# yidingjiang/action_conditioned_GANs

Hardware: AMD Instinct MI355X
Metric: GAN train steps/sec (G+D) on 64x64x3xT=8 push seq (higher is better)
Workload: dtype f32; 1 GPU; BASELINE config 2 per GPU: batch=32 64x64x3 T=8 --adv --loss bce --dna (k=5) --opt adam fp32; global_batch=32, n_critic=1, parallelism=dp1, hip_graphs=True, bn_grid_exchange=on, lookahead=True, opt=adam, trace_run=False, step_executions=1380

## Files before the change

action_conditioned_gans_amd/csrc/dna.hip:

```cpp
#include <hip/hip_runtime.h>

#include <type_traits>

#include "common.h"

namespace {

constexpr int TX = 64;

struct Second {
  void* ptr;
  int pitch, off, half;
};
__device__ __forceinline__ void second_store(const Second& s2, long long pix, int c, float v) {
  if (s2.half) reinterpret_cast<__bf16*>(s2.ptr)[pix * s2.pitch + s2.off + c] = (__bf16)v;
  else reinterpret_cast<float*>(s2.ptr)[pix * s2.pitch + s2.off + c] = v;
}
__device__ __forceinline__ void second_store_pixel(const Second& s2, long long pix, int C, const float* img_c, const float (&f)[4]) {
  if (C == 3 && s2.off == 3 && s2.pitch == 8) {
    if (s2.half) {
      typedef __bf16 bf8v __attribute__((ext_vector_type(8)));
      const bf8v v = {(__bf16)img_c[0], (__bf16)img_c[1], (__bf16)img_c[2], (__bf16)f[0], (__bf16)f[1], (__bf16)f[2], (__bf16)0.f, (__bf16)0.f};
      *reinterpret_cast<bf8v*>(reinterpret_cast<__bf16*>(s2.ptr) + pix * 8) = v;
    } else {
      float4* o = reinterpret_cast<float4*>(reinterpret_cast<float*>(s2.ptr) + pix * 8);
      o[0] = make_float4(img_c[0], img_c[1], img_c[2], f[0]);
      o[1] = make_float4(f[1], f[2], 0.f, 0.f);
    }
    return;
  }
  for (int c = 0; c < C; ++c) second_store(s2, pix, c, f[c]);
}
__device__ __forceinline__ float second_load(const Second& s2, long long pix, int c) {
  return s2.half ? (float)reinterpret_cast<const __bf16*>(s2.ptr)[pix * s2.pitch + s2.off + c]
                 : reinterpret_cast<const float*>(s2.ptr)[pix * s2.pitch + s2.off + c];
}

template <typename TL>
__host__ __device__ constexpr int logit_pitch(int kk) { return sizeof(TL) == 2 ? (kk + 7) & ~7 : kk; }

template <int K, int TY, bool BWD, int CC, typename TL>
__global__ __launch_bounds__(TX* TY) void dna_kernel(const TL* __restrict__ logits, const float* __restrict__ bias,
                                                     const float* __restrict__ img, const float* __restrict__ dout,
                                                     void* __restrict__ outv, float* __restrict__ bpart, int H, int W, int Crt,
                                                     const Second s2) {
  constexpr int KK = K * K, S = KK | 1, NT = TX * TY, P = (K - 1) / 2, LP = logit_pitch<TL>(KK);
  constexpr int WW = TX + K - 1, WH = TY + K - 1;
  constexpr bool F32 = sizeof(TL) == 4;
  __shared__ __attribute__((aligned(16))) float lg[NT * S];
  __shared__ float win[WH * WW * 4];
  __shared__ float bs[KK];
  const int C = CC ? CC : Crt;
  float* const out = reinterpret_cast<float*>(outv);
  TL* const dlog = reinterpret_cast<TL*>(outv);

  const int tid = threadIdx.x;
  const int x0 = blockIdx.x * TX, y0 = blockIdx.y * TY, b = blockIdx.z;
  const int txv = min(TX, W - x0);
  if (tid < KK) bs[tid] = bias ? bias[tid] : 0.f;

  for (int wy = tid / 64; wy < WH; wy += NT / 64) {
    const int y = y0 - P + wy;
    const bool yok = y >= 0 && y < H;
    const long long rowbase = (long long)(b * H + (yok ? y : 0)) * W * C;
    for (int f = tid % 64; f < WW * C; f += 64) {
      const int gx = (x0 - P) * C + f;
      win[wy * WW * C + f] = (yok && gx >= 0 && gx < W * C) ? img[rowbase + gx] : 0.f;
    }
  }
  const long long pix0 = (long long)(b * H + y0) * W + x0;
  const bool vec = F32 && (S == KK) && ((pix0 * KK) % 4 == 0) && (((long long)W * KK) % 4 == 0) && ((txv * KK) % 4 == 0) &&
                   ((reinterpret_cast<uintptr_t>(logits) & 15) == 0);
  if constexpr (F32) {
    if (vec) {
      const int span4 = txv * KK / 4;
      for (int ty = 0; ty < TY; ++ty) {
        if (y0 + ty >= H) break;
        const float4* src = reinterpret_cast<const float4*>(logits + (pix0 + (long long)ty * W) * KK);
        float4* dst = reinterpret_cast<float4*>(lg + ty * TX * S);
        for (int i = tid; i < span4; i += NT) dst[i] = src[i];
      }
    } else {
      for (int idx = tid; idx < TY * TX * KK; idx += NT) {
        const int ty = idx / (TX * KK), e = idx - ty * (TX * KK);
        if (y0 + ty < H && e < txv * KK) lg[(ty * TX + e / KK) * S + e % KK] = acg::ldf(logits + (pix0 + (long long)ty * W) * KK + e);
      }
    }
  } else {
    constexpr int Q = LP / 4;
    for (int idx = tid; idx < TY * TX * Q; idx += NT) {
      const int ty = idx / (TX * Q), e = idx - ty * (TX * Q), px = e / Q, q = e - px * Q;
      if (y0 + ty < H && px < txv && 4 * q < KK) {
        float v[4];
        acg::ldv<4>(logits + (pix0 + (long long)ty * W + px) * LP + 4 * q, v);
        float* d = lg + (ty * TX + px) * S + 4 * q;
#pragma unroll
        for (int u = 0; u < 4; ++u)
          if (4 * q + u < KK) d[u] = v[u];
      }
    }
  }
  __syncthreads();

  const int ty = tid / TX, tx = tid - ty * TX;
  const int y = y0 + ty, x = x0 + tx;
  const bool valid = y < H && x < W;
  float* l = lg + tid * S;
  const float* wbase = win + (ty * WW + tx) * C;

  if (valid) {
    float v[KK];
#pragma unroll
    for (int t = 0; t < KK; ++t) v[t] = l[t] + bs[t];
    float mx = v[0];
#pragma unroll
    for (int t = 1; t < KK; ++t) mx = fmaxf(mx, v[t]);
    const long long pix = (long long)(b * H + y) * W + x;
    if constexpr (!BWD) {
      float den = 0.f, a0 = 0.f, a1 = 0.f, a2 = 0.f, a3 = 0.f;
#pragma unroll
      for (int i = 0; i < K; ++i)
#pragma unroll
        for (int j = 0; j < K; ++j) {
          const float e = __expf(v[i * K + j] - mx);
          const float* wp = wbase + (i * WW + j) * C;
          den += e;
          a0 += e * wp[0];
          if (C > 1) a1 += e * wp[1];
          if (C > 2) a2 += e * wp[2];
          if (C > 3) a3 += e * wp[3];
        }
      const float inv = 1.f / den;
      float* o = out + pix * C;
      o[0] = a0 * inv;
      if (C > 1) o[1] = a1 * inv;
      if (C > 2) o[2] = a2 * inv;
      if (C > 3) o[3] = a3 * inv;
      if (s2.ptr) {
        const float fr[4] = {a0 * inv, a1 * inv, a2 * inv, a3 * inv};
        second_store_pixel(s2, pix, C, wbase + (P * WW + P) * C, fr);
      }
    } else {
      const float* dO = dout + pix * C;
      float d0 = dO[0], d1 = C > 1 ? dO[1] : 0.f, d2 = C > 2 ? dO[2] : 0.f, d3 = C > 3 ? dO[3] : 0.f;
      if (s2.ptr) {
        d0 += second_load(s2, pix, 0);
        if (C > 1) d1 += second_load(s2, pix, 1);
        if (C > 2) d2 += second_load(s2, pix, 2);
        if (C > 3) d3 += second_load(s2, pix, 3);
      }
      float gv[KK];
      float den = 0.f, dotn = 0.f;
#pragma unroll
      for (int i = 0; i < K; ++i)
#pragma unroll
        for (int j = 0; j < K; ++j) {
          const float* wp = wbase + (i * WW + j) * C;
          float g = d0 * wp[0];
          if (C > 1) g += d1 * wp[1];
          if (C > 2) g += d2 * wp[2];
          if (C > 3) g += d3 * wp[3];
          const float e = __expf(v[i * K + j] - mx);
          gv[i * K + j] = g;
          v[i * K + j] = e;
          den += e;
          dotn += e * g;
        }
      const float inv = 1.f / den, dot = dotn * inv;
#pragma unroll
      for (int t = 0; t < KK; ++t) l[t] = (v[t] * inv) * (gv[t] - dot);
    }
  } else if constexpr (BWD) {
#pragma unroll
    for (int t = 0; t < KK; ++t) l[t] = 0.f;
  }
  if constexpr (BWD) {
    __syncthreads();
    if constexpr (F32) {
      if (vec) {
        const int span4 = txv * KK / 4;
        for (int ty2 = 0; ty2 < TY; ++ty2) {
          if (y0 + ty2 >= H) break;
          float4* dstg = reinterpret_cast<float4*>(dlog + (pix0 + (long long)ty2 * W) * KK);
          const float4* srcl = reinterpret_cast<const float4*>(lg + ty2 * TX * S);
          for (int i = tid; i < span4; i += NT) dstg[i] = srcl[i];
        }
      } else {
        for (int idx = tid; idx < TY * TX * KK; idx += NT) {
          const int ty2 = idx / (TX * KK), e = idx - ty2 * (TX * KK);
          if (y0 + ty2 < H && e < txv * KK) acg::stf(dlog + (pix0 + (long long)ty2 * W) * KK + e, lg[(ty2 * TX + e / KK) * S + e % KK]);
        }
      }
    } else {
      constexpr int Q = LP / 4;
      for (int idx = tid; idx < TY * TX * Q; idx += NT) {
        const int ty2 = idx / (TX * Q), e = idx - ty2 * (TX * Q), px = e / Q, q = e - px * Q;
        if (y0 + ty2 < H && px < txv && 4 * q < KK) {
          const float* sl = lg + (ty2 * TX + px) * S + 4 * q;
          float v[4];
#pragma unroll
          for (int u = 0; u < 4; ++u) v[u] = 4 * q + u < KK ? sl[u] : 0.f;
          acg::stv<4>(dlog + (pix0 + (long long)ty2 * W + px) * LP + 4 * q, v);
        }
      }
    }
    if (bpart) {
      const int t = tid & 31, seg = tid >> 5;
      float sacc = 0.f;
      if (t < KK)
        for (int px = seg * 32; px < seg * 32 + 32; ++px) sacc += lg[px * S + t];
      __syncthreads();
      if (t < KK) win[seg * 32 + t] = sacc;
      __syncthreads();
      if (tid < KK) {
        float tot = 0.f;
        for (int g2 = 0; g2 < NT / 32; ++g2) tot += win[g2 * 32 + tid];
        bpart[(long long)((blockIdx.z * gridDim.y + blockIdx.y) * gridDim.x + blockIdx.x) * KK + tid] = tot;
      }
    }
  }
}

template <int K, bool BWD, int CC, typename TL>
__global__ __launch_bounds__(256) void dna_rows_kernel(const TL* __restrict__ logits, const float* __restrict__ bias,
                                                       const float* __restrict__ img, const float* __restrict__ dout,
                                                       void* __restrict__ outv, float* __restrict__ bpart, int H, int W, int Crt,
                                                       const Second s2) {
  constexpr int E = sizeof(TL) == 2 ? 2 : 1;
  constexpr int KK = K * K, P = (K - 1) / 2, R = (KK + 16 * E - 1) / (16 * E), WW = 64 + K - 1, LP = logit_pitch<TL>(KK);
  const int C = CC ? CC : Crt;
  __shared__ float win[K * WW * 4];
  __shared__ float bsum[BWD ? 16 * R * 16 * E : 1];
  float* const out = reinterpret_cast<float*>(outv);
  TL* const dlog = reinterpret_cast<TL*>(outv);
  const int tid = threadIdx.x, l16 = tid & 15, grp = tid >> 4;
  const int x0 = blockIdx.x * 64, y = blockIdx.y, b = blockIdx.z;
  for (int i = tid; i < K * WW * C; i += 256) {
    const int c = i % C, p = i / C, wx = p % WW, wy = p / WW;
    const int gy = y - P + wy, gx = x0 - P + wx;
    win[i] = (gy >= 0 && gy < H && gx >= 0 && gx < W) ? img[(((long long)b * H + gy) * W + gx) * C + c] : 0.f;
  }
  __syncthreads();
  auto dpp = [](float v, auto ctrl) {
    return __builtin_bit_cast(float, __builtin_amdgcn_update_dpp(0, __builtin_bit_cast(int, v), decltype(ctrl)::value, 0xF, 0xF, false));
  };
  using QP1 = std::integral_constant<int, 0xB1>;
  using QP2 = std::integral_constant<int, 0x4E>;
  using RHM = std::integral_constant<int, 0x141>;
  using RM = std::integral_constant<int, 0x140>;
  auto row_max = [&](float v) {
    v = fmaxf(v, dpp(v, QP1{})); v = fmaxf(v, dpp(v, QP2{})); v = fmaxf(v, dpp(v, RHM{})); v = fmaxf(v, dpp(v, RM{}));
    return v;
  };
  auto row_sum = [&](float v) {
    v += dpp(v, QP1{}); v += dpp(v, QP2{}); v += dpp(v, RHM{}); v += dpp(v, RM{});
    return v;
  };
  int woff[R][E];
  float bia[R][E], bacc[R][E];
#pragma unroll
  for (int r = 0; r < R; ++r)
#pragma unroll
    for (int e = 0; e < E; ++e) {
      const int t = E * (l16 + 16 * r) + e, i = t / K, j = t - i * K;
      woff[r][e] = (i * WW + j) * C;
      bia[r][e] = (bias && t < KK) ? bias[t] : 0.f;
      bacc[r][e] = 0.f;
    }
  float lall[4][R][E];
#pragma unroll
  for (int it = 0; it < 4; ++it) {
    const int x = x0 + it * 16 + grp;
    const TL* lp = logits + (((long long)b * H + y) * W + min(x, W - 1)) * LP;
#pragma unroll
    for (int r = 0; r < R; ++r) {
      const int t0 = E * (l16 + 16 * r);
      if constexpr (E == 2) {
        typedef __bf16 bf2v __attribute__((ext_vector_type(2)));
        const bf2v v = t0 < LP ? *reinterpret_cast<const bf2v*>(lp + t0) : bf2v{(__bf16)0.f, (__bf16)0.f};
        lall[it][r][0] = t0 < KK ? (float)v[0] + bia[r][0] : -3.0e38f;
        lall[it][r][1] = t0 + 1 < KK ? (float)v[1] + bia[r][1] : -3.0e38f;
      } else {
        lall[it][r][0] = t0 < KK ? acg::ldf(lp + t0) + bia[r][0] : -3.0e38f;
      }
    }
  }
#pragma unroll
  for (int it = 0; it < 4; ++it) {
    const int px = it * 16 + grp, x = x0 + px;
    if (x >= W) continue;
    const long long pix = ((long long)b * H + y) * W + x;
    float l[R][E];
    float mx = -3.0e38f;
#pragma unroll
    for (int r = 0; r < R; ++r)
#pragma unroll
      for (int e = 0; e < E; ++e) {
        l[r][e] = lall[it][r][e];
        mx = fmaxf(mx, l[r][e]);
      }
    mx = row_max(mx);
    float den = 0.f, a[4] = {0.f, 0.f, 0.f, 0.f}, d[4] = {0.f, 0.f, 0.f, 0.f};
    if constexpr (BWD) {
#pragma unroll
      for (int c = 0; c < 4; ++c) d[c] = c < C ? dout[pix * C + c] + (s2.ptr ? second_load(s2, pix, c) : 0.f) : 0.f;
    }
    float g[R][E];
#pragma unroll
    for (int r = 0; r < R; ++r)
#pragma unroll
      for (int e = 0; e < E; ++e) {
        const int t = E * (l16 + 16 * r) + e;
        const float ex = t < KK ? __expf(l[r][e] - mx) : 0.f;
        const float* wp = win + woff[r][e] + px * C;
        den += ex;
        if constexpr (!BWD) {
#pragma unroll
          for (int c = 0; c < 4; ++c)
            if (c < C) a[c] += ex * (t < KK ? wp[c] : 0.f);
        } else {
          float gg = 0.f;
          if (t < KK) {
#pragma unroll
            for (int c = 0; c < 4; ++c)
              if (c < C) gg += d[c] * wp[c];
          }
          g[r][e] = gg;
          a[0] += ex * gg;
        }
        l[r][e] = ex;
      }
    den = row_sum(den);
    const float inv = 1.f / den;
    if constexpr (!BWD) {
      float fr[4] = {0.f, 0.f, 0.f, 0.f};
#pragma unroll
      for (int c = 0; c < 4; ++c) {
        if (c < C) {
          fr[c] = row_sum(a[c]) * inv;
          if (l16 == c) out[pix * C + c] = fr[c];
        }
      }
      if (s2.ptr && l16 == 4) second_store_pixel(s2, pix, C, win + (P * WW + P + px) * C, fr);
    } else {
      const float dot = row_sum(a[0]) * inv;
      TL* op = dlog + pix * LP;
#pragma unroll
      for (int r = 0; r < R; ++r) {
        const int t0 = E * (l16 + 16 * r);
        float dv[E];
#pragma unroll
        for (int e = 0; e < E; ++e) {
          dv[e] = t0 + e < KK ? l[r][e] * inv * (g[r][e] - dot) : 0.f;
          bacc[r][e] += dv[e];
        }
        if constexpr (E == 2) {
          typedef __bf16 bf2v __attribute__((ext_vector_type(2)));
          if (t0 < KK) *reinterpret_cast<bf2v*>(op + t0) = bf2v{(__bf16)dv[0], (__bf16)dv[1]};
        } else {
          if (t0 < KK) acg::stf(op + t0, dv[0]);
        }
      }
    }
  }
  if constexpr (BWD) {
    if (bpart) {
#pragma unroll
      for (int r = 0; r < R; ++r)
#pragma unroll
        for (int e = 0; e < E; ++e) bsum[grp * (R * 16 * E) + E * (l16 + 16 * r) + e] = bacc[r][e];
      __syncthreads();
      if (tid < KK) {
        float tot = 0.f;
        for (int g2 = 0; g2 < 16; ++g2) tot += bsum[g2 * (R * 16 * E) + tid];
        bpart[(long long)((blockIdx.z * gridDim.y + blockIdx.y) * gridDim.x + blockIdx.x) * KK + tid] = tot;
      }
    }
  }
}

constexpr int kSegs = 32;
__global__ __launch_bounds__(256) void dna_dbias_sum(const float* __restrict__ part, float* __restrict__ out, float acc, int KK, int nrows) {
  __shared__ double sh[256];
  const int cl = threadIdx.x & 31, rl = threadIdx.x >> 5, c = blockIdx.x * 32 + cl;
  const int per = (nrows + gridDim.y - 1) / gridDim.y, r0 = blockIdx.y * per, r1 = min(nrows, r0 + per);
  double s2 = 0.0;
  if (c < KK) {
#pragma unroll 4
    for (int b2 = r0 + rl; b2 < r1; b2 += 8) s2 += part[(long long)b2 * KK + c];
  }
  sh[threadIdx.x] = s2;
  __syncthreads();
  if (rl == 0 && c < KK) {
#pragma unroll
    for (int r = 1; r < 8; ++r) s2 += sh[r * 32 + cl];
    float* o = out + (long long)blockIdx.y * KK + c;
    *o = (acc != 0.f ? acc * *o : 0.f) + (float)s2;
  }
}

#ifndef ACG_DNA_ROWS_MIN
#define ACG_DNA_ROWS_MIN 6
#endif

#ifndef ACG_DNA_TY
#define ACG_DNA_TY 4
#endif
dim3 dna_grid(int k, int B, int H, int W) {
  if (k >= ACG_DNA_ROWS_MIN) return dim3((W + 63) / 64, H, B);
  return dim3((W + TX - 1) / TX, (H + ACG_DNA_TY - 1) / ACG_DNA_TY, B);
}

template <int K, bool BWD, typename TL>
int launch_k(const TL* logits, const float* bias, const float* img, const float* dout, void* out, float* bpart, int B, int H, int W,
             int C, hipStream_t st, const Second& s2) {
  const dim3 grid = dna_grid(K, B, H, W);
  if constexpr (K >= ACG_DNA_ROWS_MIN) {
    if (C == 3) ACG_LAUNCH((dna_rows_kernel<K, BWD, 3, TL>), grid, dim3(256), 0, st, logits, bias, img, dout, out, bpart, H, W, C, s2);
    else ACG_LAUNCH((dna_rows_kernel<K, BWD, 0, TL>), grid, dim3(256), 0, st, logits, bias, img, dout, out, bpart, H, W, C, s2);
  } else {
    constexpr int TY = ACG_DNA_TY;
    if (C == 3) ACG_LAUNCH((dna_kernel<K, TY, BWD, 3, TL>), grid, dim3(TX * TY), 0, st, logits, bias, img, dout, out, bpart, H, W, C, s2);
    else ACG_LAUNCH((dna_kernel<K, TY, BWD, 0, TL>), grid, dim3(TX * TY), 0, st, logits, bias, img, dout, out, bpart, H, W, C, s2);
  }
  return acg::check_launch(BWD ? "dna_bwd" : "dna_fwd");
}

template <bool BWD, typename TL>
int dispatch(int k, const void* logits, const float* bias, const float* img, const float* dout, void* out, float* bpart, int B, int H,
             int W, int C, hipStream_t st, const Second& s2) {
  switch (k) {
#define ACG_DNA_CASE(KV) case KV: return launch_k<KV, BWD, TL>((const TL*)logits, bias, img, dout, out, bpart, B, H, W, C, st, s2);
    ACG_DNA_CASE(1) ACG_DNA_CASE(2) ACG_DNA_CASE(3) ACG_DNA_CASE(4) ACG_DNA_CASE(5) ACG_DNA_CASE(6)
    ACG_DNA_CASE(7) ACG_DNA_CASE(8) ACG_DNA_CASE(9) ACG_DNA_CASE(10) ACG_DNA_CASE(11)
#undef ACG_DNA_CASE
    default: return acg::fail(ACG_ERR_UNSUPPORTED, "dna: ksize %d outside 1..11", k);
  }
}

int check(const char* who, int B, int H, int W, int C, int k, int dtype) {
  ACG_REQUIRE(dtype == ACG_F32 || dtype == ACG_BF16, ACG_ERR_UNSUPPORTED, "%s: dtype %d", who, dtype);
  ACG_REQUIRE(B > 0 && H > 0 && W > 0, ACG_ERR_INVALID_ARG, "%s: non-positive size", who);
  ACG_REQUIRE(C >= 1 && C <= 4, ACG_ERR_INVALID_ARG, "%s: channels %d outside 1..4", who, C);
  ACG_REQUIRE(B <= 65535 && H <= 65535, ACG_ERR_UNSUPPORTED, "%s: grid too large", who);
  ACG_REQUIRE((long long)B * H * W * ((k * k + 7) & ~7) < 2147483647ll, ACG_ERR_UNSUPPORTED, "%s: tensor exceeds 2^31 elements", who);
  return ACG_OK;
}

}

extern "C" {

size_t acg_dna_workspace_bytes(int32_t B, int32_t H, int32_t W, int32_t k) {
  if (B <= 0 || H <= 0 || W <= 0 || k < 1 || k > 11) return 0;
  const dim3 g = dna_grid(k, B, H, W);
  return ((size_t)g.x * g.y * g.z + kSegs) * (size_t)(k * k) * sizeof(float);
}

namespace {
int second_of(const char* who, const void* ptr, int pitch, int off, int dt, int C, Second* s2) {
  s2->ptr = const_cast<void*>(ptr); s2->pitch = pitch; s2->off = off; s2->half = dt == ACG_BF16;
  if (!ptr) return ACG_OK;
  ACG_REQUIRE(dt == ACG_F32 || dt == ACG_BF16, ACG_ERR_UNSUPPORTED, "%s: second tensor dtype %d", who, dt);
  ACG_REQUIRE(off >= 0 && pitch >= off + C, ACG_ERR_INVALID_ARG, "%s: second tensor: %d channels at offset %d do not fit pitch %d", who, C, off, pitch);
  return ACG_OK;
}
}

int32_t acg_dna_fwd(const void* logits, const float* bias, const void* image, void* out, void* out2, int32_t out2_pitch,
                    int32_t out2_offset, int32_t out2_dtype, int32_t B, int32_t H, int32_t W, int32_t C, int32_t k, int32_t dtype,
                    acg_stream_t stream) {
  if (int rc = check("dna_fwd", B, H, W, C, k, dtype)) return rc;
  ACG_REQUIRE(logits && image && out, ACG_ERR_INVALID_ARG, "dna_fwd: null pointer");
  Second s2;
  if (int rc = second_of("dna_fwd", out2, out2_pitch, out2_offset, out2_dtype, C, &s2)) return rc;
  if (dtype == ACG_BF16) return dispatch<false, __bf16>(k, logits, bias, (const float*)image, nullptr, out, nullptr, B, H, W, C, acg::to_stream(stream), s2);
  return dispatch<false, float>(k, logits, bias, (const float*)image, nullptr, out, nullptr, B, H, W, C, acg::to_stream(stream), s2);
}

int32_t acg_dna_bwd(const void* logits, const float* bias, const void* image, const void* dout, const void* dout2, int32_t dout2_pitch,
                    int32_t dout2_offset, int32_t dout2_dtype, void* dlogits, float* dbias, float dbias_acc, int32_t B, int32_t H,
                    int32_t W, int32_t C, int32_t k, int32_t dtype, void* ws, size_t wsb, acg_stream_t stream) {
  if (int rc = check("dna_bwd", B, H, W, C, k, dtype)) return rc;
  ACG_REQUIRE(logits && image && dout && dlogits, ACG_ERR_INVALID_ARG, "dna_bwd: null pointer");
  Second s2;
  if (int rc = second_of("dna_bwd", dout2, dout2_pitch, dout2_offset, dout2_dtype, C, &s2)) return rc;
  ACG_REQUIRE(!dbias || (ws && wsb >= acg_dna_workspace_bytes(B, H, W, k)), ACG_ERR_WORKSPACE, "dna_bwd: workspace too small for dbias");
  hipStream_t st = acg::to_stream(stream);
  float* bpart = dbias ? (float*)ws : nullptr;
  int rc;
  if (dtype == ACG_BF16) rc = dispatch<true, __bf16>(k, logits, bias, (const float*)image, (const float*)dout, dlogits, bpart, B, H, W, C, st, s2);
  else rc = dispatch<true, float>(k, logits, bias, (const float*)image, (const float*)dout, dlogits, bpart, B, H, W, C, st, s2);
  if (rc || !dbias) return rc;
  const dim3 g = dna_grid(k, B, H, W);
  const int nblk = (int)(g.x * g.y * g.z), KK = k * k, tb = (KK + 31) / 32;
  if (nblk <= 1024) {
    ACG_LAUNCH(dna_dbias_sum, dim3(tb, 1), dim3(256), 0, st, (const float*)bpart, dbias, dbias_acc, KK, nblk);
  } else {
    float* seg = bpart + (size_t)nblk * KK;
    ACG_LAUNCH(dna_dbias_sum, dim3(tb, kSegs), dim3(256), 0, st, (const float*)bpart, seg, 0.f, KK, nblk);
    ACG_LAUNCH(dna_dbias_sum, dim3(tb, 1), dim3(256), 0, st, (const float*)seg, dbias, dbias_acc, KK, kSegs);
  }
  return acg::check_launch("dna_dbias_sum");
}

}
```

Baseline: 461.0 steps/s (batch-32 G+D steps, all ranks).

## Make DNA kernel persistent with double-buffered register-prefetched tile loads

Turns the small-kernel DNA forward/backward into a persistent grid-stride kernel capped at about two blocks per CU. Each block prefetches the next tile's image window, logits and upstream gradients into registers while it computes the current tile, then stages them into a second shared-memory buffer. This hides global-load latency behind the softmax-weighted accumulation. It also unrolls the dbias partial-sum reduction and picks the vector path at launch time. In exchange it uses more registers and shared memory, and with only 2x CUs blocks it may lose occupancy and parallelism on small inputs.

```diff
diff --git a/action_conditioned_gans_amd/csrc/dna.hip b/action_conditioned_gans_amd/csrc/dna.hip
--- a/action_conditioned_gans_amd/csrc/dna.hip
+++ b/action_conditioned_gans_amd/csrc/dna.hip
@@ -1,5 +1,7 @@
 #include <hip/hip_runtime.h>
 
+#include <algorithm>
+#include <cstdlib>
 #include <type_traits>
 
 #include "common.h"
@@ -35,189 +37,302 @@
   return s2.half ? (float)reinterpret_cast<const __bf16*>(s2.ptr)[pix * s2.pitch + s2.off + c]
                  : reinterpret_cast<const float*>(s2.ptr)[pix * s2.pitch + s2.off + c];
 }
+__device__ __forceinline__ unsigned second_load_raw(const Second& s2, long long pix, int c) {
+  return s2.half ? (unsigned)reinterpret_cast<const unsigned short*>(s2.ptr)[pix * s2.pitch + s2.off + c]
+                 : reinterpret_cast<const unsigned*>(s2.ptr)[pix * s2.pitch + s2.off + c];
+}
+__device__ __forceinline__ float second_value(const Second& s2, unsigned raw) { return __uint_as_float(s2.half ? raw << 16 : raw); }
 
 template <typename TL>
 __host__ __device__ constexpr int logit_pitch(int kk) { return sizeof(TL) == 2 ? (kk + 7) & ~7 : kk; }
 
-template <int K, int TY, bool BWD, int CC, typename TL>
-__global__ __launch_bounds__(TX* TY) void dna_kernel(const TL* __restrict__ logits, const float* __restrict__ bias,
+struct Tile {
+  int x0, y0, b;
+};
+__device__ __forceinline__ Tile tile_at(int t, int tiles_x, int tiles_y, int ty) {
+  const int row = t / tiles_x, b = row / tiles_y;
+  return Tile{(t - row * tiles_x) * TX, (row - b * tiles_y) * ty, b};
+}
+
+template <int K, int TY, bool BWD, int CC, typename TL, bool VEC>
+__global__ __launch_bounds__(TX* TY, 2) void dna_kernel(const TL* __restrict__ logits, const float* __restrict__ bias,
                                                      const float* __restrict__ img, const float* __restrict__ dout,
                                                      void* __restrict__ outv, float* __restrict__ bpart, int H, int W, int Crt,
-                                                     const Second s2) {
+                                                     int tiles_x, int tiles_y, int ntiles, const Second s2) {
   constexpr int KK = K * K, S = KK | 1, NT = TX * TY, P = (K - 1) / 2, LP = logit_pitch<TL>(KK);
-  constexpr int WW = TX + K - 1, WH = TY + K - 1;
+  constexpr int WW = TX + K - 1, WH = TY + K - 1, CM = CC ? CC : 4;
   constexpr bool F32 = sizeof(TL) == 4;
-  __shared__ __attribute__((aligned(16))) float lg[NT * S];
-  __shared__ float win[WH * WW * 4];
+  static_assert(TX == 64 && (!VEC || (F32 && S == KK)), "dna_kernel: a tile row is one wave; float4 spans need the linear layout");
+  constexpr int WR = (WH + TY - 1) / TY, WC = (WW * CM + 63) / 64, NV = (TX * KK / 4 + NT - 1) / NT, Q = LP / 4;
+  constexpr int NL = VEC ? TY * NV * 4 : F32 ? KK : Q * 2;
+  __shared__ __attribute__((aligned(16))) float lg[2][NT * S];
+  __shared__ float win[2][WH * WW * CM];
+  __shared__ float dl[BWD ? 2 : 1][BWD ? NT * CM : 1];
+  __shared__ float cs[BWD ? NT : 1];
   __shared__ float bs[KK];
   const int C = CC ? CC : Crt;
   float* const out = reinterpret_cast<float*>(outv);
   TL* const dlog = reinterpret_cast<TL*>(outv);
 
-  const int tid = threadIdx.x;
-  const int x0 = blockIdx.x * TX, y0 = blockIdx.y * TY, b = blockIdx.z;
-  const int txv = min(TX, W - x0);
+  const int tid = threadIdx.x, ty = tid / TX, tx = tid - ty * TX;
   if (tid < KK) bs[tid] = bias ? bias[tid] : 0.f;
-
-  for (int wy = tid / 64; wy < WH; wy += NT / 64) {
-    const int y = y0 - P + wy;
-    const bool yok = y >= 0 && y < H;
-    const long long rowbase = (long long)(b * H + (yok ? y : 0)) * W * C;
-    for (int f = tid % 64; f < WW * C; f += 64) {
-      const int gx = (x0 - P) * C + f;
-      win[wy * WW * C + f] = (yok && gx >= 0 && gx < W * C) ? img[rowbase + gx] : 0.f;
-    }
-  }
-  const long long pix0 = (long long)(b * H + y0) * W + x0;
-  const bool vec = F32 && (S == KK) && ((pix0 * KK) % 4 == 0) && (((long long)W * KK) % 4 == 0) && ((txv * KK) % 4 == 0) &&
-                   ((reinterpret_cast<uintptr_t>(logits) & 15) == 0);
-  if constexpr (F32) {
-    if (vec) {
+  float wr[WR][WC], lr[NL], dn[4] = {0.f, 0.f, 0.f, 0.f};
+  unsigned du[4] = {0u, 0u, 0u, 0u};
+
+  auto load = [&](const Tile& T, bool on) {
+    const int txv = min(TX, W - T.x0);
+    const long long pix0 = (long long)(T.b * H + T.y0) * W + T.x0;
+    if constexpr (BWD) {
+      const long long pix = (long long)(T.b * H + min(T.y0 + ty, H - 1)) * W + min(T.x0 + tx, W - 1);
+      const float* dO = dout + pix * C;
+      dn[0] = dO[0];
+      if (C > 1) dn[1] = dO[1];
+      if (C > 2) dn[2] = dO[2];
+      if (C > 3) dn[3] = dO[3];
+      if (s2.ptr) {
+        du[0] = second_load_raw(s2, pix, 0);
+        if (C > 1) du[1] = second_load_raw(s2, pix, 1);
+        if (C > 2) du[2] = second_load_raw(s2, pix, 2);
+        if (C > 3) du[3] = second_load_raw(s2, pix, 3);
+      }
+    }
+#pragma unroll
+    for (int r = 0; r < WR; ++r) {
+      const int wy = ty + r * TY, y = T.y0 - P + wy;
+      const bool yok = on && wy < WH && y >= 0 && y < H;
+      const long long rowbase = (long long)(T.b * H + (yok ? y : 0)) * W * C;
+#pragma unroll
+      for (int c = 0; c < WC; ++c) {
+        const int f = tx + c * 64, gx = (T.x0 - P) * C + f;
+        wr[r][c] = 0.f;
+        if (yok && f < WW * C && gx >= 0 && gx < W * C) wr[r][c] = img[rowbase + gx];
+      }
+    }
+    if constexpr (VEC) {
       const int span4 = txv * KK / 4;
-      for (int ty = 0; ty < TY; ++ty) {
-        if (y0 + ty >= H) break;
-        const float4* src = reinterpret_cast<const float4*>(logits + (pix0 + (long long)ty * W) * KK);
-        float4* dst = reinterpret_cast<float4*>(lg + ty * TX * S);
-        for (int i = tid; i < span4; i += NT) dst[i] = src[i];
+#pragma unroll
+      for (int r = 0; r < TY; ++r) {
+        const float4* src = reinterpret_cast<const float4*>(logits + (pix0 + (long long)r * W) * KK);
+#pragma unroll
+        for (int n = 0; n < NV; ++n) {
+          const int i = tid + n * NT;
+          float4 v = make_float4(0.f, 0.f, 0.f, 0.f);
+          if (on && T.y0 + r < H && i < span4) v = src[i];
+          float* d = lr + (r * NV + n) * 4;
+          d[0] = v.x; d[1] = v.y; d[2] = v.z; d[3] = v.w;
+        }
+      }
+    } else if constexpr (F32) {
+#pragma unroll
+      for (int n = 0; n < KK; ++n) {
+        const int idx = tid + n * NT, r = idx / (TX * KK), e = idx - r * (TX * KK);
+        lr[n] = 0.f;
+        if (on && T.y0 + r < H && e < txv * KK) lr[n] = acg::ldf(logits + (pix0 + (long long)r * W) * KK + e);
       }
     } else {
-      for (int idx = tid; idx < TY * TX * KK; idx += NT) {
-        const int ty = idx / (TX * KK), e = idx - ty * (TX * KK);
-        if (y0 + ty < H && e < txv * KK) lg[(ty * TX + e / KK) * S + e % KK] = acg::ldf(logits + (pix0 + (long long)ty * W) * KK + e);
-      }
-    }
-  } else {
-    constexpr int Q = LP / 4;
-    for (int idx = tid; idx < TY * TX * Q; idx += NT) {
-      const int ty = idx / (TX * Q), e = idx - ty * (TX * Q), px = e / Q, q = e - px * Q;
-      if (y0 + ty < H && px < txv && 4 * q < KK) {
-        float v[4];
-        acg::ldv<4>(logits + (pix0 + (long long)ty * W + px) * LP + 4 * q, v);
-        float* d = lg + (ty * TX + px) * S + 4 * q;
-#pragma unroll
-        for (int u = 0; u < 4; ++u)
-          if (4 * q + u < KK) d[u] = v[u];
-      }
-    }
-  }
+#pragma unroll
+      for (int n = 0; n < Q; ++n) {
+        const int idx = tid + n * NT, r = idx / (TX * Q), e = idx - r * (TX * Q), px = e / Q, q = e - px * Q;
+        uint2 v = make_uint2(0u, 0u);
+        if (on && T.y0 + r < H && px < txv && 4 * q < KK) v = *reinterpret_cast<const uint2*>(logits + (pix0 + (long long)r * W + px) * LP + 4 * q);
+        lr[n * 2] = __uint_as_float(v.x);
+        lr[n * 2 + 1] = __uint_as_float(v.y);
+      }
+    }
+  };
+  auto stage = [&](const Tile& T, int st, bool on) {
+    int tid = threadIdx.x;
+    asm volatile("" : "+v"(tid));
+    const int ty = tid / TX, tx = tid - ty * TX;
+    const int txv = min(TX, W - T.x0);
+    if constexpr (BWD) {
+      if (on && T.y0 + ty < H && T.x0 + tx < W) {
+#pragma unroll
+        for (int c = 0; c < CM; ++c)
+          if (c < C) dl[st][tid * CM + c] = s2.ptr ? dn[c] + second_value(s2, du[c]) : dn[c];
+      }
+    }
+#pragma unroll
+    for (int r = 0; r < WR; ++r) {
+      const int wy = ty + r * TY;
+#pragma unroll
+      for (int c = 0; c < WC; ++c) {
+        const int f = tx + c * 64;
+        if (on && wy < WH && f < WW * C) win[st][wy * WW * C + f] = wr[r][c];
+      }
+    }
+    if constexpr (VEC) {
+      const int span4 = txv * KK / 4;
+#pragma unroll
+      for (int r = 0; r < TY; ++r) {
+        float4* dst = reinterpret_cast<float4*>(lg[st] + r * TX * S);
+#pragma unroll
+        for (int n = 0; n < NV; ++n) {
+          const int i = tid + n * NT;
+          const float* d = lr + (r * NV + n) * 4;
+          if (on && T.y0 + r < H && i < span4) dst[i] = make_float4(d[0], d[1], d[2], d[3]);
+        }
+      }
+    } else if constexpr (F32) {
+#pragma unroll
+      for (int n = 0; n < KK; ++n) {
+        const int idx = tid + n * NT, r = idx / (TX * KK), e = idx - r * (TX * KK);
+        if (on && T.y0 + r < H && e < txv * KK) lg[st][(r * TX + e / KK) * S + e % KK] = lr[n];
+      }
+    } else {
+#pragma unroll
+      for (int n = 0; n < Q; ++n) {
+        const int idx = tid + n * NT, r = idx / (TX * Q), e = idx - r * (TX * Q), px = e / Q, q = e - px * Q;
+        if (on && T.y0 + r < H && px < txv && 4 * q < KK) {
+          float* d = lg[st] + (r * TX + px) * S + 4 * q;
+          const unsigned lo = __float_as_uint(lr[n * 2]), hi = __float_as_uint(lr[n * 2 + 1]);
+          const float v[4] = {__uint_as_float(lo << 16), __uint_as_float(lo & 0xffff0000u), __uint_as_float(hi << 16), __uint_as_float(hi & 0xffff0000u)};
+#pragma unroll
+          for (int u = 0; u < 4; ++u)
+            if (4 * q + u < KK) d[u] = v[u];
+        }
+      }
+    }
+  };
+
+  int tile = blockIdx.x;
+  Tile cur = tile_at(tile, tiles_x, tiles_y, TY);
+  load(cur, true);
+  stage(cur, 0, true);
   __syncthreads();
 
-  const int ty = tid / TX, tx = tid - ty * TX;
-  const int y = y0 + ty, x = x0 + tx;
-  const bool valid = y < H && x < W;
-  float* l = lg + tid * S;
-  const float* wbase = win + (ty * WW + tx) * C;
-
-  if (valid) {
-    float v[KK];
-#pragma unroll
-    for (int t = 0; t < KK; ++t) v[t] = l[t] + bs[t];
-    float mx = v[0];
-#pragma unroll
-    for (int t = 1; t < KK; ++t) mx = fmaxf(mx, v[t]);
+  for (int st = 0; tile < ntiles; st ^= 1) {
+    const int ntile = tile + (int)gridDim.x;
+    const bool more = ntile < ntiles;
+    const Tile nxt = tile_at(more ? ntile : tile, tiles_x, tiles_y, TY);
+    load(nxt, more);
+
+    const int x0 = cur.x0, y0 = cur.y0, b = cur.b;
+    const int y = y0 + ty, x = x0 + tx;
+    const bool valid = y < H && x < W;
     const long long pix = (long long)(b * H + y) * W + x;
+    float* l = lg[st] + tid * S;
+    const float* wbase = win[st] + (ty * WW + tx) * C;
+    float fr[4] = {0.f, 0.f, 0.f, 0.f};
+
+    if (valid) {
+      float v[KK];
+#pragma unroll
+      for (int t = 0; t < KK; ++t) v[t] = l[t] + bs[t];
+      float mx = v[0];
+#pragma unroll
+      for (int t = 1; t < KK; ++t) mx = fmaxf(mx, v[t]);
+      if constexpr (!BWD) {
+        float den = 0.f, a0 = 0.f, a1 = 0.f, a2 = 0.f, a3 = 0.f;
+#pragma unroll
+        for (int i = 0; i < K; ++i)
+#pragma unroll
+          for (int j = 0; j < K; ++j) {
+            const float e = __expf(v[i * K + j] - mx);
+            const float* wp = wbase + (i * WW + j) * C;
+            den += e;
+            if constexpr (CC == 3) {
+              a0 = fmaf(e, wp[0], a0);
+              a1 = fmaf(e, wp[1], a1);
+              a2 = fmaf(e, wp[2], a2);
+            } else {
+              a0 += e * wp[0];
+              if (C > 1) a1 += e * wp[1];
+              if (C > 2) a2 += e * wp[2];
+              if (C > 3) a3 += e * wp[3];
+            }
+          }
+        const float inv = 1.f / den;
+        fr[0] = a0 * inv; fr[1] = a1 * inv; fr[2] = a2 * inv; fr[3] = a3 * inv;
+      } else {
+        const float* dO = dl[st] + tid * CM;
+        const float d0 = dO[0], d1 = C > 1 ? dO[1] : 0.f, d2 = C > 2 ? dO[2] : 0.f, d3 = C > 3 ? dO[3] : 0.f;
+        float gv[KK];
+        float den = 0.f, dotn = 0.f;
+#pragma unroll
+        for (int i = 0; i < K; ++i)
+#pragma unroll
+          for (int j = 0; j < K; ++j) {
+            const float* wp = wbase + (i * WW + j) * C;
+            float g = d0 * wp[0];
+            if (C > 1) g += d1 * wp[1];
+            if (C > 2) g += d2 * wp[2];
+            if (C > 3) g += d3 * wp[3];
+            const float e = __expf(v[i * K + j] - mx);
+            gv[i * K + j] = g;
+            v[i * K + j] = e;
+            den += e;
+            dotn += e * g;
+          }
+        const float inv = 1.f / den, dot = dotn * inv;
+#pragma unroll
+        for (int t = 0; t < KK; ++t) l[t] = (v[t] * inv) * (gv[t] - dot);
+      }
+    } else if constexpr (BWD) {
+#pragma unroll
+      for (int t = 0; t < KK; ++t) l[t] = 0.f;
+    }
+    if constexpr (BWD) __syncthreads();
+
+    stage(nxt, st ^ 1, more);
+    __builtin_amdgcn_s_waitcnt(0x0F70);
+
     if constexpr (!BWD) {
-      float den = 0.f, a0 = 0.f, a1 = 0.f, a2 = 0.f, a3 = 0.f;
-#pragma unroll
-      for (int i = 0; i < K; ++i)
-#pragma unroll
-        for (int j = 0; j < K; ++j) {
-          const float e = __expf(v[i * K + j] - mx);
-          const float* wp = wbase + (i * WW + j) * C;
-          den += e;
-          a0 += e * wp[0];
-          if (C > 1) a1 += e * wp[1];
-          if (C > 2) a2 += e * wp[2];
-          if (C > 3) a3 += e * wp[3];
-        }
-      const float inv = 1.f / den;
-      float* o = out + pix * C;
-      o[0] = a0 * inv;
-      if (C > 1) o[1] = a1 * inv;
-      if (C > 2) o[2] = a2 * inv;
-      if (C > 3) o[3] = a3 * inv;
-      if (s2.ptr) {
-        const float fr[4] = {a0 * inv, a1 * inv, a2 * inv, a3 * inv};
-        second_store_pixel(s2, pix, C, wbase + (P * WW + P) * C, fr);
+      if (valid) {
+        float* o = out + pix * C;
+        o[0] = fr[0];
+        if (C > 1) o[1] = fr[1];
+        if (C > 2) o[2] = fr[2];
+        if (C > 3) o[3] = fr[3];
+        if (s2.ptr) second_store_pixel(s2, pix, C, wbase + (P * WW + P) * C, fr);
       }
     } else {
-      const float* dO = dout + pix * C;
-      float d0 = dO[0], d1 = C > 1 ? dO[1] : 0.f, d2 = C > 2 ? dO[2] : 0.f, d3 = C > 3 ? dO[3] : 0.f;
-      if (s2.ptr) {
-        d0 += second_load(s2, pix, 0);
-        if (C > 1) d1 += second_load(s2, pix, 1);
-        if (C > 2) d2 += second_load(s2, pix, 2);
-        if (C > 3) d3 += second_load(s2, pix, 3);
-      }
-      float gv[KK];
-      float den = 0.f, dotn = 0.f;
-#pragma unroll
-      for (int i = 0; i < K; ++i)
-#pragma unroll
-        for (int j = 0; j < K; ++j) {
-          const float* wp = wbase + (i * WW + j) * C;
-          float g = d0 * wp[0];
-          if (C > 1) g += d1 * wp[1];
-          if (C > 2) g += d2 * wp[2];
-          if (C > 3) g += d3 * wp[3];
-          const float e = __expf(v[i * K + j] - mx);
-          gv[i * K + j] = g;
-          v[i * K + j] = e;
-          den += e;
-          dotn += e * g;
-        }
-      const float inv = 1.f / den, dot = dotn * inv;
-#pragma unroll
-      for (int t = 0; t < KK; ++t) l[t] = (v[t] * inv) * (gv[t] - dot);
-    }
-  } else if constexpr (BWD) {
-#pragma unroll
-    for (int t = 0; t < KK; ++t) l[t] = 0.f;
-  }
-  if constexpr (BWD) {
-    __syncthreads();
-    if constexpr (F32) {
-      if (vec) {
+      const int txv = min(TX, W - x0);
+      const long long pix0 = (long long)(b * H + y0) * W + x0;
+      if constexpr (VEC) {
         const int span4 = txv * KK / 4;
         for (int ty2 = 0; ty2 < TY; ++ty2) {
           if (y0 + ty2 >= H) break;
           float4* dstg = reinterpret_cast<float4*>(dlog + (pix0 + (long long)ty2 * W) * KK);
-          const float4* srcl = reinterpret_cast<const float4*>(lg + ty2 * TX * S);
+          const float4* srcl = reinterpret_cast<const float4*>(lg[st] + ty2 * TX * S);
           for (int i = tid; i < span4; i += NT) dstg[i] = srcl[i];
         }
-      } else {
+      } else if constexpr (F32) {
         for (int idx = tid; idx < TY * TX * KK; idx += NT) {
           const int ty2 = idx / (TX * KK), e = idx - ty2 * (TX * KK);
-          if (y0 + ty2 < H && e < txv * KK) acg::stf(dlog + (pix0 + (long long)ty2 * W) * KK + e, lg[(ty2 * TX + e / KK) * S + e % KK]);
-        }
-      }
-    } else {
-      constexpr int Q = LP / 4;
-      for (int idx = tid; idx < TY * TX * Q; idx += NT) {
-        const int ty2 = idx / (TX * Q), e = idx - ty2 * (TX * Q), px = e / Q, q = e - px * Q;
-        if (y0 + ty2 < H && px < txv && 4 * q < KK) {
-          const float* sl = lg + (ty2 * TX + px) * S + 4 * q;
-          float v[4];
-#pragma unroll
-          for (int u = 0; u < 4; ++u) v[u] = 4 * q + u < KK ? sl[u] : 0.f;
-          acg::stv<4>(dlog + (pix0 + (long long)ty2 * W + px) * LP + 4 * q, v);
-        }
-      }
-    }
-    if (bpart) {
-      const int t = tid & 31, seg = tid >> 5;
-      float sacc = 0.f;
-      if (t < KK)
-        for (int px = seg * 32; px < seg * 32 + 32; ++px) sacc += lg[px * S + t];
-      __syncthreads();
-      if (t < KK) win[seg * 32 + t] = sacc;
-      __syncthreads();
-      if (tid < KK) {
+          if (y0 + ty2 < H && e < txv * KK) acg::stf(dlog + (pix0 + (long long)ty2 * W) * KK + e, lg[st][(ty2 * TX + e / KK) * S + e % KK]);
+        }
+      } else {
+        for (int idx = tid; idx < TY * TX * Q; idx += NT) {
+          const int ty2 = idx / (TX * Q), e = idx - ty2 * (TX * Q), px = e / Q, q = e - px * Q;
+          if (y0 + ty2 < H && px < txv && 4 * q < KK) {
+            const float* sl = lg[st] + (ty2 * TX + px) * S + 4 * q;
+            float v[4];
+#pragma unroll
+            for (int u = 0; u < 4; ++u) v[u] = 4 * q + u < KK ? sl[u] : 0.f;
+            acg::stv<4>(dlog + (pix0 + (long long)ty2 * W + px) * LP + 4 * q, v);
+          }
+        }
+      }
+      if (bpart) {
+        const int t = tid & 31, seg = tid >> 5;
+        if (t < KK) {
+          float sacc = 0.f;
+          for (int px = seg * 32; px < seg * 32 + 32; ++px) sacc += lg[st][px * S + t];
+          cs[seg * 32 + t] = sacc;
+        }
+      }
+    }
+    __syncthreads();
+    if constexpr (BWD) {
+      if (bpart && tid < KK) {
         float tot = 0.f;
-        for (int g2 = 0; g2 < NT / 32; ++g2) tot += win[g2 * 32 + tid];
-        bpart[(long long)((blockIdx.z * gridDim.y + blockIdx.y) * gridDim.x + blockIdx.x) * KK + tid] = tot;
-      }
-    }
+        for (int g2 = 0; g2 < NT / 32; ++g2) tot += cs[g2 * 32 + tid];
+        bpart[(long long)tile * KK + tid] = tot;
+      }
+    }
+    cur = nxt;
+    tile = ntile;
   }
 }
 
@@ -379,15 +494,21 @@
   }
 }
 
-constexpr int kSegs = 32;
+constexpr int kSegs = 32, kSumU = 16;
 __global__ __launch_bounds__(256) void dna_dbias_sum(const float* __restrict__ part, float* __restrict__ out, float acc, int KK, int nrows) {
   __shared__ double sh[256];
   const int cl = threadIdx.x & 31, rl = threadIdx.x >> 5, c = blockIdx.x * 32 + cl;
   const int per = (nrows + gridDim.y - 1) / gridDim.y, r0 = blockIdx.y * per, r1 = min(nrows, r0 + per);
   double s2 = 0.0;
   if (c < KK) {
-#pragma unroll 4
-    for (int b2 = r0 + rl; b2 < r1; b2 += 8) s2 += part[(long long)b2 * KK + c];
+    for (int b2 = r0 + rl; b2 < r1; b2 += 8 * kSumU) {
+      float v[kSumU];
+#pragma unroll
+      for (int u = 0; u < kSumU; ++u) v[u] = part[(long long)min(b2 + 8 * u, r1 - 1) * KK + c];
+#pragma unroll
+      for (int u = 0; u < kSumU; ++u)
+        if (b2 + 8 * u < r1) s2 += v[u];
+    }
   }
   sh[threadIdx.x] = s2;
   __syncthreads();
@@ -409,6 +530,21 @@
 dim3 dna_grid(int k, int B, int H, int W) {
   if (k >= ACG_DNA_ROWS_MIN) return dim3((W + 63) / 64, H, B);
   return dim3((W + TX - 1) / TX, (H + ACG_DNA_TY - 1) / ACG_DNA_TY, B);
+}
+
+int env_int(const char* name, int dflt) {
+  const char* v = getenv(name);
+  return (v && *v) ? atoi(v) : dflt;
+}
+int device_cus() {
+  static const int ncu = [] { int dev = 0, n = 0; if (hipGetDevice(&dev) != hipSuccess || hipDeviceGetAttribute(&n, hipDeviceAttributeMultiprocessorCount, dev) != hipSuccess) n = 0; (void)hipGetLastError(); return n; }();
+  return ncu;
+}
+int dna_blocks(int tiles) {
+  static const int max_blocks = env_int("ACG_DNA_MAX_BLOCKS", 0);
+  const int ncu = device_cus();
+  const int cap = max_blocks > 0 ? max_blocks : ncu > 0 ? 2 * ncu : tiles;
+  return std::max(1, std::min(tiles, cap));
 }
 
 template <int K, bool BWD, typename TL>
@@ -419,9 +555,24 @@
     if (C == 3) ACG_LAUNCH((dna_rows_kernel<K, BWD, 3, TL>), grid, dim3(256), 0, st, logits, bias, img, dout, out, bpart, H, W, C, s2);
     else ACG_LAUNCH((dna_rows_kernel<K, BWD, 0, TL>), grid, dim3(256), 0, st, logits, bias, img, dout, out, bpart, H, W, C, s2);
   } else {
-    constexpr int TY = ACG_DNA_TY;
-    if (C == 3) ACG_LAUNCH((dna_kernel<K, TY, BWD, 3, TL>), grid, dim3(TX * TY), 0, st, logits, bias, img, dout, out, bpart, H, W, C, s2);
-    else ACG_LAUNCH((dna_kernel<K, TY, BWD, 0, TL>), grid, dim3(TX * TY), 0, st, logits, bias, img, dout, out, bpart, H, W, C, s2);
+    constexpr int TY = ACG_DNA_TY, KK = K * K;
+    const int tiles = (int)(grid.x * grid.y * grid.z);
+    const dim3 blocks(dna_blocks(tiles));
+#define ACG_DNA_GO(CCV, VECV) \
+  ACG_LAUNCH((dna_kernel<K, TY, BWD, CCV, TL, VECV>), blocks, dim3(TX * TY), 0, st, logits, bias, img, dout, out, bpart, H, W, C, (int)grid.x, (int)grid.y, tiles, s2)
+    bool vec = false;
+    if constexpr (sizeof(TL) == 4 && (KK & 1)) {
+      vec = ((long long)W * KK) % 4 == 0 && (reinterpret_cast<uintptr_t>(logits) & 15) == 0 && (!BWD || (reinterpret_cast<uintptr_t>(out) & 15) == 0);
+      if (vec) {
+        if (C == 3) ACG_DNA_GO(3, true);
+        else ACG_DNA_GO(0, true);
+      }
+    }
+    if (!vec) {
+      if (C == 3) ACG_DNA_GO(3, false);
+      else ACG_DNA_GO(0, false);
+    }
+#undef ACG_DNA_GO
   }
   return acg::check_launch(BWD ? "dna_bwd" : "dna_fwd");
 }
```

Result: no change. 462.0 steps/s (batch-32 G+D steps, all ranks), median of 6 (+0.2%).
